# XMUDM/SPEX

Measured on NVIDIA B200. Metric: lightgcn_propagation_gedges_per_s, higher is better.
Workload: dtype f32

## Files before the change

spex_b200/csrc/spmm.cu:

```cuda
#include "common.cuh"
#include <math.h>

namespace spex {

int64_t g_launches = 0;

template <int D>
struct RowShape {
  static_assert(D == 32 || D == 64 || D == 128, "vector path supports D in {32,64,128}");
  static constexpr int LPR = D / 4;
  static constexpr int G = 32 / LPR;
};

template <int D, int U, bool kList, bool kHot = false>
__device__ __forceinline__ float4 warp_row_accumulate(const int32_t* __restrict__ col,
                                                      const float* __restrict__ val,
                                                      const float* __restrict__ X, int64_t start,
                                                      int64_t end, int lane) {
  constexpr int LPR = RowShape<D>::LPR, G = RowShape<D>::G;
  const int grp = lane / LPR, sub = lane % LPR;
  const float* Xs = X + sub * 4;
  float4 acc = f4_zero();
  uint64_t pol_last = 0, pol_first = 0;
  if (kHot) {
// ... 99 lines not shown
      f8 x[U];
      float vv[U];
#pragma unroll
      for (int u = 0; u < U; ++u) {
        const int cc = __shfl_sync(kFull, c, k0 + u, LPR8);
        vv[u] = __shfl_sync(kFull, v, k0 + u, LPR8);
        if (k0 + u < ng) {
          x[u] = gather_row8<D, kHot, kCold>(Xs, cc);
        } else {
          x[u].a = f4_zero();
          x[u].b = f4_zero();
          vv[u] = 0.f;
        }
      }
#pragma unroll
      for (int u = 0; u < U; ++u) f8_fma(acc, vv[u], x[u]);
    }
  }
}

template <int D>
__device__ __forceinline__ void groups_reduce8(f8& acc) {
#pragma unroll
  for (int m = D / 8; m < 32; m <<= 1) {
    f4_add(acc.a, f4_shfl_xor(acc.a, m));
    f4_add(acc.b, f4_shfl_xor(acc.b, m));
  }
}

template <int D, int U, bool kHot>
__device__ __forceinline__ float4 warp_row_accumulate8(const int32_t* __restrict__ col,
                                                       const float* __restrict__ val,
                                                       const float* __restrict__ X, int64_t start,
                                                       int64_t end, int lane) {
  constexpr int LPR8 = D / 8;
  const int grp = lane / LPR8, sub = lane % LPR8;
  const float* Xs = X + sub * 8;
  f8 acc;
  acc.a = f4_zero();
  acc.b = f4_zero();
  int rem = (int)(end - start);
  const int32_t* cp = col + start + lane;
  const float* vp = val + start + lane;
  int c = 0;
  float v = 0.f;
  if (lane < rem) {
    c = ld_stream_s32(cp);
    v = ld_stream_f32(vp);
  }
  while (rem > 0) {
    int cn = 0;
    float vn = 0.f;
    if (lane + 32 < rem) {
      cn = ld_stream_s32(cp + 32);
      vn = ld_stream_f32(vp + 32);
    }
    batch_accumulate8<D, U, kHot>(acc, Xs, c, v, rem, grp);
    c = cn;
    v = vn;
    cp += 32;
    vp += 32;
    rem -= 32;
  }
  groups_reduce8<D>(acc);
  const int src = (lane >> 1) & (LPR8 - 1);
  float4 lo, hi;
  lo.x = __shfl_sync(kFull, acc.a.x, src);
  lo.y = __shfl_sync(kFull, acc.a.y, src);
  lo.z = __shfl_sync(kFull, acc.a.z, src);
  lo.w = __shfl_sync(kFull, acc.a.w, src);
  hi.x = __shfl_sync(kFull, acc.b.x, src);
  hi.y = __shfl_sync(kFull, acc.b.y, src);
  hi.z = __shfl_sync(kFull, acc.b.z, src);
  hi.w = __shfl_sync(kFull, acc.b.w, src);
  return (lane & 1) ? hi : lo;
}

#ifndef SPEX_V8_U
#define SPEX_V8_U 4
#endif
#ifndef SPEX_MASK_U
#define SPEX_MASK_U 2
#endif
#ifndef SPEX_V8_MINB
#define SPEX_V8_MINB 32
#endif
template <int D, bool kHot>
__device__ __forceinline__ float4 warp_row_accumulate8_masked(const int32_t* __restrict__ col,
                                                              const float* __restrict__ val,
                                                              const float* __restrict__ X,
                                                              const uint8_t* __restrict__ nz, int64_t start,
                                                              int64_t end, int lane) {
  constexpr int LPR8 = D / 8;
  constexpr int U = SPEX_MASK_U;
  const int grp = lane / LPR8, sub = lane % LPR8;
  const float* Xs = X + sub * 8;
  f8 acc;
  acc.a = f4_zero();
  acc.b = f4_zero();
  int rem = (int)(end - start);
  const int32_t* cp = col + start + lane;
  const float* vp = val + start + lane;
  constexpr uint32_t kIdMask = kHot ? 0x7fffffffu : 0xffffffffu;
  int c = 0, cn = 0;
  float v = 0.f, vn = 0.f;
  bool on = false;
  if (lane < rem) {
    c = ld_stream_s32(cp);
    v = ld_stream_f32(vp);
  }
  if (lane + 32 < rem) {
    cn = ld_stream_s32(cp + 32);
    vn = ld_stream_f32(vp + 32);
  }
  if (lane < rem) on = nz[(uint32_t)c & kIdMask] != 0;
  while (rem > 0) {
    int c2 = 0;
    float v2 = 0.f;
    if (lane + 64 < rem) {
      c2 = ld_stream_s32(cp + 64);
      v2 = ld_stream_f32(vp + 64);
    }
    bool onn = false;
    if (lane + 32 < rem) onn = nz[(uint32_t)cn & kIdMask] != 0;
    const unsigned act = __ballot_sync(kFull, on);
    unsigned mine = (act >> (grp * LPR8)) & (LPR8 == 32 ? 0xffffffffu : ((1u << LPR8) - 1u));
#pragma unroll 1
    while (__any_sync(kFull, mine != 0)) {
      f8 x[U];
      float vv[U];
#pragma unroll
      for (int u = 0; u < U; ++u) {
        const bool has = mine != 0;
        const int src = grp * LPR8 + (has ? __ffs(mine) - 1 : 0);
        mine &= mine - 1;
        const int cc = __shfl_sync(kFull, c, src);
        vv[u] = __shfl_sync(kFull, v, src);
        if (has) {
          x[u] = gather_row8<D, kHot>(Xs, cc);
        } else {
          x[u].a = f4_zero();
          x[u].b = f4_zero();
          vv[u] = 0.f;
        }
      }
#pragma unroll
      for (int u = 0; u < U; ++u) f8_fma(acc, vv[u], x[u]);
    }
    c = cn;
    v = vn;
    on = onn;
    cn = c2;
    vn = v2;
    cp += 32;
    vp += 32;
    rem -= 32;
  }
#pragma unroll
  for (int m = LPR8; m < 32; m <<= 1) {
    f4_add(acc.a, f4_shfl_xor(acc.a, m));
    f4_add(acc.b, f4_shfl_xor(acc.b, m));
  }
  const int src = (lane >> 1) & (LPR8 - 1);
  float4 lo, hi;
  lo.x = __shfl_sync(kFull, acc.a.x, src);
  lo.y = __shfl_sync(kFull, acc.a.y, src);
  lo.z = __shfl_sync(kFull, acc.a.z, src);
  lo.w = __shfl_sync(kFull, acc.a.w, src);
  hi.x = __shfl_sync(kFull, acc.b.x, src);
  hi.y = __shfl_sync(kFull, acc.b.y, src);
  hi.z = __shfl_sync(kFull, acc.b.z, src);
  hi.w = __shfl_sync(kFull, acc.b.w, src);
  return (lane & 1) ? hi : lo;
}

template <int D, int U, bool kHot, bool kV8, bool kMask = false>
__device__ __forceinline__ float4 row_sum(const int32_t* __restrict__ col, const float* __restrict__ val,
                                          const float* __restrict__ X, int64_t start, int64_t end, int lane,
                                          const uint8_t* __restrict__ nz = nullptr) {
  if (kV8 && kMask) return warp_row_accumulate8_masked<D, kHot>(col, val, X, nz, start, end, lane);
  if (kV8) return warp_row_accumulate8<D, (D >= 64 ? SPEX_V8_U : D / 8), kHot>(col, val, X, start, end, lane);
  return warp_row_accumulate<D, U, false, kHot>(col, val, X, start, end, lane);
}

struct Epilogue {
  float* Y;
  const float* addend;
  float addend_scale;
  float* Z;
  float z_scale;
  float* peer[8];
  int n_peers;
  int64_t peer_row_offset;
  float* mcast;
  const float* pub_src;
  float* pub_mcast;
  float* pub_peer[8];
  int n_pub_peers;
  float* adam_p;
  float* adam_m;
  float* adam_v;
  float adam_b1, adam_b2, adam_eps, adam_step_size, adam_bc2_sqrt;
};

__device__ __forceinline__ void adam_update(float& pp, float gg, float& mm, float& vv, const Epilogue& ep) {
  mm = mm + (gg - mm) * (1.f - ep.adam_b1);
  vv = vv * ep.adam_b2 + (1.f - ep.adam_b2) * gg * gg;
  const float denom = sqrtf(vv) / ep.adam_bc2_sqrt + ep.adam_eps;
  pp = pp - ep.adam_step_size * (mm / denom);
}

template <int D>
__device__ __forceinline__ void row_epilogue(const Epilogue& ep, float4 acc, int64_t row, int lane) {
  constexpr int LPR = RowShape<D>::LPR;
  if (lane < LPR) {
    const int64_t off = row * D + lane * 4;
    if (ep.Y) *reinterpret_cast<float4*>(ep.Y + off) = acc;
    if (ep.mcast) {
      st_multimem_f4(ep.mcast + (row + ep.peer_row_offset) * D + lane * 4, acc);
    } else if (ep.n_peers > 0) {
      const int64_t poff = (row + ep.peer_row_offset) * D + lane * 4;
#pragma unroll
      for (int p = 0; p < 8; ++p)
        if (p < ep.n_peers) *reinterpret_cast<float4*>(ep.peer[p] + poff) = acc;
    }
    float4 z = acc;
    if (ep.Z || ep.adam_p) {
      float4 a = f4_zero();
      if (ep.addend) a = ld_f4(ep.addend + off);
      z.x = (a.x * ep.addend_scale + acc.x) * ep.z_scale;
      z.y = (a.y * ep.addend_scale + acc.y) * ep.z_scale;
      z.z = (a.z * ep.addend_scale + acc.z) * ep.z_scale;
      z.w = (a.w * ep.addend_scale + acc.w) * ep.z_scale;
      if (ep.Z) *reinterpret_cast<float4*>(ep.Z + off) = z;
    }
    float4 pnew = f4_zero();
    if (ep.adam_p) {
      pnew = ld_f4(ep.adam_p + off);
      float4 mm = ld_f4(ep.adam_m + off), vv = ld_f4(ep.adam_v + off);
      adam_update(pnew.x, z.x, mm.x, vv.x, ep);
      adam_update(pnew.y, z.y, mm.y, vv.y, ep);
      adam_update(pnew.z, z.z, mm.z, vv.z, ep);
      adam_update(pnew.w, z.w, mm.w, vv.w, ep);
      *reinterpret_cast<float4*>(ep.adam_p + off) = pnew;
      *reinterpret_cast<float4*>(ep.adam_m + off) = mm;
      *reinterpret_cast<float4*>(ep.adam_v + off) = vv;
    }
    if (ep.pub_src || (ep.adam_p && (ep.pub_mcast || ep.n_pub_peers > 0))) {
      const float4 v = ep.adam_p ? pnew : ld_stream_f4(ep.pub_src + off);
      const int64_t poff = (row + ep.peer_row_offset) * D + lane * 4;
      if (ep.pub_mcast) {
        st_multimem_f4(ep.pub_mcast + poff, v);
      } else {
#pragma unroll
        for (int p = 0; p < 8; ++p)
          if (p < ep.n_pub_peers) *reinterpret_cast<float4*>(ep.pub_peer[p] + poff) = v;
      }
    }
  }
}

#ifndef SPEX_ROWS_PER_CTA
#define SPEX_ROWS_PER_CTA 1
#endif
#ifndef SPEX_U64
#define SPEX_U64 8
#endif
constexpr int kRowsPerCta = SPEX_ROWS_PER_CTA;

template <int D, int U, bool kHot, bool kV8, bool kMask>
__global__ void __launch_bounds__(kRowsPerCta * 32, SPEX_V8_MINB / kRowsPerCta)
spmm_rows_kernel(const int64_t* __restrict__ rowptr, const int32_t* __restrict__ col,
                 const float* __restrict__ val, const float* __restrict__ X, int64_t n_rows,
                 int32_t skip_longer_than, Epilogue ep, const int32_t* __restrict__ row_sel,
                 const uint8_t* __restrict__ nz) {
  const int lane = threadIdx.x & 31;
  int64_t row = (int64_t)blockIdx.x * kRowsPerCta + (threadIdx.x >> 5);
  if (row >= n_rows) return;
  if (row_sel) row = row_sel[row];
  const int64_t start = rowptr[row], end = rowptr[row + 1];
  if (skip_longer_than > 0 && end > start + skip_longer_than) return;
  if (kMask && ep.addend && lane < RowShape<D>::LPR && (lane & 7) == 0)
    asm volatile("prefetch.global.L2 [%0];" ::"l"(ep.addend + row * D + lane * 4));
  const float4 acc = row_sum<D, U, kHot, kV8, kMask>(col, val, X, start, end, lane, nz);
  row_epilogue<D>(ep, acc, row, lane);
}

template <int D, int U, bool kHot, bool kV8, bool kMask>
__global__ void __launch_bounds__(kRowsPerCta * 32, SPEX_V8_MINB / kRowsPerCta)
spmm_seg_list_kernel(const int32_t* __restrict__ col, const float* __restrict__ val,
                     const float* __restrict__ X, const int64_t* __restrict__ seg_start,
                     const int32_t* __restrict__ seg_count, int32_t n_seg, float* __restrict__ partial,
                     const int32_t* __restrict__ seg_sel, const uint8_t* __restrict__ nz) {
  constexpr int LPR = RowShape<D>::LPR;
  const int lane = threadIdx.x & 31;
  int seg = blockIdx.x * kRowsPerCta + (threadIdx.x >> 5);
  if (seg >= n_seg) return;
  if (seg_sel) seg = seg_sel[seg];
  const int64_t start = seg_start[seg];
  const float4 acc = row_sum<D, U, kHot, kV8, kMask>(col, val, X, start, start + seg_count[seg], lane, nz);
  if (lane < LPR) *reinterpret_cast<float4*>(partial + (int64_t)seg * D + lane * 4) = acc;
}

#ifndef SPEX_SEG_HUB_RUN
#define SPEX_SEG_HUB_RUN 8
#endif
#ifndef SPEX_SEG_MID_RUN
#define SPEX_SEG_MID_RUN 2
#endif
constexpr int kHubRun = SPEX_SEG_HUB_RUN, kMidRun = SPEX_SEG_MID_RUN;
static_assert(kHubRun <= 32 && kMidRun <= 32, "a run's segment extents are held one per lane");

template <int D, bool kHot, bool kCold>
__device__ __forceinline__ void seg_run8(const int32_t* __restrict__ col, const float* __restrict__ val,
                                         const float* __restrict__ X, const int64_t* __restrict__ seg_start,
                                         const int32_t* __restrict__ seg_count, int first, int n,
                                         float* __restrict__ partial, int lane) {
  constexpr int LPR8 = D / 8, U = D >= 64 ? SPEX_V8_U : D / 8;
  const int grp = lane / LPR8, sub = lane % LPR8;
  const float* Xs = X + sub * 8;
  int64_t my_start = 0;
  int my_cnt = 0;
  if (lane < n) {
    my_start = seg_start[first + lane];
    my_cnt = seg_count[first + lane];
  }
  int64_t start = __shfl_sync(kFull, my_start, 0);
  int rem = __shfl_sync(kFull, my_cnt, 0);
  int c = 0;
  float v = 0.f;
  if (lane < rem) {
    c = ld_stream_s32(col + start + lane);
    v = ld_stream_f32(val + start + lane);
  }
#pragma unroll 1
  for (int k = 0; k < n; ++k) {
    const int64_t nstart = __shfl_sync(kFull, my_start, (k + 1) & 31);
    const int ncnt = k + 1 < n ? __shfl_sync(kFull, my_cnt, (k + 1) & 31) : 0;
    f8 acc;
    acc.a = f4_zero();
    acc.b = f4_zero();
    int64_t e = start + lane;
#pragma unroll 1
    while (rem > 0) {
      int cn = 0;
      float vn = 0.f;
      if (rem > 32) {
        if (lane + 32 < rem) {
          cn = ld_stream_s32(col + e + 32);
          vn = ld_stream_f32(val + e + 32);
        }
      } else if (lane < ncnt) {
        cn = ld_stream_s32(col + nstart + lane);
        vn = ld_stream_f32(val + nstart + lane);
      }
      batch_accumulate8<D, U, kHot, kCold>(acc, Xs, c, v, rem, grp);
      c = cn;
      v = vn;
      e += 32;
      rem -= 32;
    }
    groups_reduce8<D>(acc);
    if (lane < LPR8) {
      float* p = partial + (int64_t)(first + k) * D + lane * 8;
      st_stream_f4(p, acc.a);
      st_stream_f4(p + 4, acc.b);
    }
    start = nstart;
    rem = ncnt;
  }
}

template <int D, bool kHot>
__global__ void __launch_bounds__(32, SPEX_V8_MINB)
spmm_seg_runs_kernel(const int32_t* __restrict__ col, const float* __restrict__ val, const float* __restrict__ X,
                     const int64_t* __restrict__ seg_start, const int32_t* __restrict__ seg_count, int32_t n_seg,
                     int32_t n_hub_seg, float* __restrict__ partial) {
  const int lane = threadIdx.x;
  const int hub_warps = (n_hub_seg + kHubRun - 1) / kHubRun;
  const int w = blockIdx.x;
  if (w < hub_warps) {
    const int first = w * kHubRun;
    const int n = min(kHubRun, n_hub_seg - first);
    seg_run8<D, kHot, false>(col, val, X, seg_start, seg_count, first, n, partial, lane);
  } else {
    const int first = n_hub_seg + (w - hub_warps) * kMidRun;
    if (first >= n_seg) return;
    const int n = min(kMidRun, n_seg - first);
    seg_run8<D, kHot, kHot>(col, val, X, seg_start, seg_count, first, n, partial, lane);
  }
}

template <int D, int U>
__global__ void __launch_bounds__(kRowsPerCta * 32)
spmm_long_fix_list_kernel(const int32_t* __restrict__ long_rows,
                          const int32_t* __restrict__ long_segptr, const int32_t* __restrict__ row_seg,
                          int32_t n_long, const float* __restrict__ partial, Epilogue ep,
                          const int32_t* __restrict__ slot_sel) {
  const int lane = threadIdx.x & 31;
  int r = blockIdx.x * kRowsPerCta + (threadIdx.x >> 5);
  if (r >= n_long) return;
  if (slot_sel) r = slot_sel[r];
  const float4 acc = warp_row_accumulate<D, U, true>(row_seg, nullptr, partial, long_segptr[r],
                                                     long_segptr[r + 1], lane);
  row_epilogue<D>(ep, acc, (int64_t)long_rows[r], lane);
}

template <int NV>
__global__ void __launch_bounds__(kRowsPerCta * 32)
spmm_rows_generic_kernel(const int64_t* __restrict__ rowptr, const int32_t* __restrict__ col,
                         const float* __restrict__ val, const float* __restrict__ X,
                         int64_t n_rows, int32_t D, Epilogue ep) {
  const int lane = threadIdx.x & 31;
  const int64_t row = (int64_t)blockIdx.x * kRowsPerCta + (threadIdx.x >> 5);
  if (row >= n_rows) return;
  const int64_t start = rowptr[row], end = rowptr[row + 1];
  float4 acc[NV];
#pragma unroll
  for (int v = 0; v < NV; ++v) acc[v] = f4_zero();
  for (int64_t base = start; base < end; base += 32) {
    const int64_t e = base + lane;
    int c = 0;
    float w = 0.f;
    if (e < end) {
      c = ld_stream_s32(col + e);
      w = ld_stream_f32(val + e);
    }
    const int n = (int)((end - base) < 32 ? (end - base) : 32);
    for (int j = 0; j < n; ++j) {
      const int cc = __shfl_sync(kFull, c, j);
      const float ww = __shfl_sync(kFull, w, j);
#pragma unroll
      for (int v = 0; v < NV; ++v) {
        const int d = (lane + 32 * v) * 4;
        if (d < D) f4_fma(acc[v], ww, ld_gather_f4(X + (int64_t)cc * D + d));
      }
    }
  }
#pragma unroll
  for (int v = 0; v < NV; ++v) {
    const int d = (lane + 32 * v) * 4;
    if (d < D) {
      const int64_t off = row * D + d;
      if (ep.Y) *reinterpret_cast<float4*>(ep.Y + off) = acc[v];
      if (ep.mcast) {
        st_multimem_f4(ep.mcast + (row + ep.peer_row_offset) * D + d, acc[v]);
      } else {
        for (int p = 0; p < ep.n_peers; ++p)
          *reinterpret_cast<float4*>(ep.peer[p] + (row + ep.peer_row_offset) * D + d) = acc[v];
      }
      if (ep.Z) {
        float4 a = f4_zero();
        if (ep.addend) a = ld_f4(ep.addend + off);
        float4 z;
        z.x = (a.x * ep.addend_scale + acc[v].x) * ep.z_scale;
        z.y = (a.y * ep.addend_scale + acc[v].y) * ep.z_scale;
        z.z = (a.z * ep.addend_scale + acc[v].z) * ep.z_scale;
        z.w = (a.w * ep.addend_scale + acc[v].w) * ep.z_scale;
        *reinterpret_cast<float4*>(ep.Z + off) = z;
      }
    }
  }
}

static bool g_rows_only = false;

struct RowSubset {
  const int32_t* rows;
  int64_t n_rows;
  const int32_t* long_slots;
  int32_t n_long;
  const int32_t* seg_ids;
  int32_t n_seg;
};

template <int D, int U, bool kHot, bool kV8, bool kMask>
static int launch_vec_h(const int64_t* rowptr, const int32_t* col, const float* val, const float* X,
                        int64_t n_rows, const Epilogue& ep, const spex_long_plan* plan,
                        cudaStream_t st, const RowSubset* sub, const uint8_t* nz) {
  const bool rows_only = g_rows_only;
  const bool has_long = plan && plan->n_long > 0;
  const int64_t n_work = sub ? sub->n_rows : n_rows;
  const int64_t grid = (n_work + kRowsPerCta - 1) / kRowsPerCta;
  if (grid > 0x7fffffffLL) return SPEX_E_TOOBIG;
  if (grid > 0) {
    spmm_rows_kernel<D, U, kHot, kV8, kMask><<<(unsigned)grid, kRowsPerCta * 32, 0, st>>>(
        rowptr, col, val, X, n_work, has_long ? plan->seg_len : 0, ep, sub ? sub->rows : nullptr, nz);
    count_launch();
  }
  if (rows_only) return check_last();
  if (has_long) {
    const int32_t n_seg = sub ? sub->n_seg : plan->n_seg;
    const int32_t n_long = sub ? sub->n_long : plan->n_long;
    const int32_t* seg_sel = sub ? sub->seg_ids : nullptr;
    const int32_t* slot_sel = sub ? sub->long_slots : nullptr;
    if (n_long == 0) return check_last();
    const int gs = (n_seg + kRowsPerCta - 1) / kRowsPerCta;
    const int gf = (n_long + kRowsPerCta - 1) / kRowsPerCta;
    if (kV8 && !kMask && !sub && plan->n_hub_seg > 0) {
      const int n_mid = n_seg - plan->n_hub_seg;
      const int gr = (plan->n_hub_seg + kHubRun - 1) / kHubRun + (n_mid + kMidRun - 1) / kMidRun;
      spmm_seg_runs_kernel<D, kHot><<<gr, 32, 0, st>>>(col, val, X, plan->seg_start, plan->seg_count, n_seg,
                                                       plan->n_hub_seg, plan->partial);
    } else {
      spmm_seg_list_kernel<D, U, kHot, kV8, kMask><<<gs, kRowsPerCta * 32, 0, st>>>(
          col, val, X, plan->seg_start, plan->seg_count, n_seg, plan->partial, seg_sel, nz);
    }
    spmm_long_fix_list_kernel<D, U><<<gf, kRowsPerCta * 32, 0, st>>>(
        plan->long_rows, plan->long_segptr, plan->row_seg, n_long, plan->partial, ep, slot_sel);
    count_launch(2);
  }
  return check_last();
}

template <int D, int U>
static int launch_vec(const int64_t* rowptr, const int32_t* col, const float* val, const float* X,
                      int64_t n_rows, const Epilogue& ep, const spex_long_plan* plan,
                      cudaStream_t st, const RowSubset* sub, const uint8_t* nz) {
  const bool v8 = (reinterpret_cast<uintptr_t>(X) & 31u) == 0;
  const bool hot = plan && (plan->flags & SPEX_PLAN_COL_HOTBIT);
  if (nz && v8) {
    if (hot) return launch_vec_h<D, U, true, true, true>(rowptr, col, val, X, n_rows, ep, plan, st, sub, nz);
    return launch_vec_h<D, U, false, true, true>(rowptr, col, val, X, n_rows, ep, plan, st, sub, nz);
  }
  if (hot) {
    if (v8) return launch_vec_h<D, U, true, true, false>(rowptr, col, val, X, n_rows, ep, plan, st, sub, nullptr);
    return launch_vec_h<D, U, true, false, false>(rowptr, col, val, X, n_rows, ep, plan, st, sub, nullptr);
  }
  if (v8) return launch_vec_h<D, U, false, true, false>(rowptr, col, val, X, n_rows, ep, plan, st, sub, nullptr);
  return launch_vec_h<D, U, false, false, false>(rowptr, col, val, X, n_rows, ep, plan, st, sub, nullptr);
}

int spmm_launch(const int64_t* rowptr, const int32_t* col, const float* val, const float* X,
                int64_t n_rows, int32_t D, const Epilogue& ep, const spex_long_plan* plan,
                cudaStream_t st, const RowSubset* sub = nullptr, const uint8_t* nz = nullptr) {
  SPEX_RETURN_IF(!rowptr || !X || n_rows < 0, SPEX_E_BADARG);
  SPEX_RETURN_IF(n_rows > 0 && (!col || !val), SPEX_E_BADARG);
  SPEX_RETURN_IF(D <= 0 || (D & 3) || D > 512, SPEX_E_BADDIM);
  SPEX_RETURN_IF(!aligned16(X) || !aligned16(ep.Y) || !aligned16(ep.Z) || !aligned16(ep.addend),
                 SPEX_E_ALIGN);
  SPEX_RETURN_IF(plan && (plan->flags & ~SPEX_PLAN_COL_HOTBIT), SPEX_E_BADARG);
  if (plan && plan->n_long > 0) {
    SPEX_RETURN_IF(plan->seg_len < 32 || !plan->long_rows || !plan->long_segptr ||
                       !plan->partial || plan->n_seg < plan->n_long,
                   SPEX_E_BADARG);
    SPEX_RETURN_IF(!plan->seg_start || !plan->seg_count || !plan->row_seg, SPEX_E_BADARG);
    SPEX_RETURN_IF(plan->n_hub_seg < 0 || plan->n_hub_seg > plan->n_seg, SPEX_E_BADARG);
    SPEX_RETURN_IF(!aligned16(plan->partial), SPEX_E_ALIGN);
  }
  if (n_rows == 0) return 0;
  switch (D) {
    case 32: return launch_vec<32, 4>(rowptr, col, val, X, n_rows, ep, plan, st, sub, nz);
    case 64: return launch_vec<64, SPEX_U64>(rowptr, col, val, X, n_rows, ep, plan, st, sub, nz);
    case 128: return launch_vec<128, 8>(rowptr, col, val, X, n_rows, ep, plan, st, sub, nz);
    default: break;
  }
  SPEX_RETURN_IF(sub != nullptr, SPEX_E_BADDIM);
  SPEX_RETURN_IF(plan && (plan->flags & SPEX_PLAN_COL_HOTBIT), SPEX_E_BADDIM);
  SPEX_RETURN_IF(ep.pub_src != nullptr || ep.adam_p != nullptr, SPEX_E_BADDIM);
  const int64_t grid = (n_rows + kRowsPerCta - 1) / kRowsPerCta;
  if (grid > 0x7fffffffLL) return SPEX_E_TOOBIG;
  const int nv = (D + 127) / 128;
  switch (nv) {
    case 1: spmm_rows_generic_kernel<1><<<(unsigned)grid, kRowsPerCta * 32, 0, st>>>(rowptr, col, val, X, n_rows, D, ep); break;
    case 2: spmm_rows_generic_kernel<2><<<(unsigned)grid, kRowsPerCta * 32, 0, st>>>(rowptr, col, val, X, n_rows, D, ep); break;
    case 3: spmm_rows_generic_kernel<3><<<(unsigned)grid, kRowsPerCta * 32, 0, st>>>(rowptr, col, val, X, n_rows, D, ep); break;
    default: spmm_rows_generic_kernel<4><<<(unsigned)grid, kRowsPerCta * 32, 0, st>>>(rowptr, col, val, X, n_rows, D, ep); break;
  }
  count_launch();
  return check_last();
}

__global__ void copy_f4_kernel(const float4* __restrict__ src, float4* __restrict__ dst, int64_t n4) {
  int64_t i = (int64_t)blockIdx.x * blockDim.x + threadIdx.x;
  const int64_t stride = (int64_t)gridDim.x * blockDim.x;
  for (; i < n4; i += stride) dst[i] = src[i];
}

struct PeerTables {
  float* peer[8];
  int n_peers;
};
__global__ void __launch_bounds__(256)
push_rows_kernel(const float4* __restrict__ src, int64_t n4, int64_t dst_off4, PeerTables pt) {
  int64_t i = (int64_t)blockIdx.x * blockDim.x + threadIdx.x;
  const int64_t stride = (int64_t)gridDim.x * blockDim.x;
  const int rot = blockIdx.x % pt.n_peers;
  for (; i < n4; i += stride) {
    const float4 v = ld_stream_f4(reinterpret_cast<const float*>(src + i));
#pragma unroll
    for (int p = 0; p < 8; ++p) {
      if (p < pt.n_peers) {
        int q = p + rot;
        if (q >= pt.n_peers) q -= pt.n_peers;
        reinterpret_cast<float4*>(pt.peer[q])[dst_off4 + i] = v;
      }
    }
  }
}

__global__ void __launch_bounds__(256)
mcast_rows_kernel(const float4* __restrict__ src, int64_t n4, float* __restrict__ mcast_dst) {
  int64_t i = (int64_t)blockIdx.x * blockDim.x + threadIdx.x;
  const int64_t stride = (int64_t)gridDim.x * blockDim.x;
  for (; i < n4; i += stride)
    st_multimem_f4(mcast_dst + 4 * i, ld_stream_f4(reinterpret_cast<const float*>(src + i)));
}

__global__ void gather_scale_kernel(const float* __restrict__ src, const int64_t* __restrict__ idx,
                                    const float* __restrict__ scale, float divisor,
                                    float* __restrict__ out, int64_t n) {
  int64_t i = (int64_t)blockIdx.x * blockDim.x + threadIdx.x;
  const int64_t stride = (int64_t)gridDim.x * blockDim.x;
  for (; i < n; i += stride) {
    float v = idx ? src[idx[i]] : src[i];
    if (scale) v *= scale[i];
    if (divisor != 1.f) v = v / divisor;
    out[i] = v;
  }
}

__device__ __forceinline__ uint32_t edge_draw(uint64_t seed, uint32_t r, uint32_t c) {
  return (uint32_t)(splitmix64(seed ^ (((uint64_t)r << 32) | c)) >> 40);
}

constexpr int kDropChunk = 1024;
constexpr int kDropUnroll = 4;

template <bool kT, bool kTpos>
__global__ void __launch_bounds__(256)
edge_dropout_kernel(const int64_t* __restrict__ rowptr, const int32_t* __restrict__ col,
                    const float* __restrict__ val, const int64_t* __restrict__ tpos, int64_t n_rows,
                    int64_t row_offset, uint64_t seed, float keep_prob, float* __restrict__ val_out,
                    float* __restrict__ valT_out) {
  uint32_t k_min = 0, k_hi = 1u << 24;
  while (k_min < k_hi) {
    const uint32_t mid = (k_min + k_hi) >> 1;
    if (__float2int_rz(__fadd_rn(__uint2float_rn(mid) * 0x1p-24f, keep_prob)) != 0) k_hi = mid; else k_min = mid + 1;
  }
  const bool divide = keep_prob != 1.f;
  const int lane = threadIdx.x & (kWarp - 1);
  const int64_t warps = (int64_t)gridDim.x * (blockDim.x / kWarp);
  const int64_t e_end = __ldg(rowptr + n_rows);
  for (int64_t c0 = __ldg(rowptr) + ((int64_t)blockIdx.x * (blockDim.x / kWarp) + threadIdx.x / kWarp) * kDropChunk;
       c0 < e_end; c0 += warps * kDropChunk) {
    int64_t lo = 0, hi = n_rows;
    while (hi - lo > 1) {
      const int64_t mid = (lo + hi) >> 1;
      if (__ldg(rowptr + mid) <= c0) lo = mid; else hi = mid;
    }
    int64_t row = lo;
    int32_t row_end = (int32_t)(__ldg(rowptr + row + 1) - c0);
    const int n = (int)min((int64_t)kDropChunk, e_end - c0);
    const int32_t* cc = col + c0;
    const float* vc = val + c0;
    float* oc = val_out + c0;
    float* ot = kT ? valT_out + c0 : nullptr;
    for (int i0 = lane; i0 < n; i0 += kDropUnroll * kWarp) {
      uint32_t cv[kDropUnroll];
      float v[kDropUnroll], vt[kDropUnroll];
#pragma unroll
      for (int k = 0; k < kDropUnroll; ++k) {
        const int i = i0 + k * kWarp;
        if (i < n) {
          cv[k] = (uint32_t)ld_stream_s32(cc + i) & 0x7fffffffu;
          v[k] = ld_stream_f32(vc + i);
          if (kT && kTpos) vt[k] = __ldg(val + __ldcs(tpos + c0 + i));
        }
      }
#pragma unroll
      for (int k = 0; k < kDropUnroll; ++k) {
        const int i = i0 + k * kWarp;
        if (i >= n) break;
        while (row_end <= i) row_end = (int32_t)(__ldg(rowptr + (++row) + 1) - c0);
        const uint32_t r = (uint32_t)(row + row_offset);
        const float q = divide ? v[k] / keep_prob : v[k];
        __stcs(oc + i, edge_draw(seed, r, cv[k]) >= k_min ? q : v[k] * 0.f);
        if (kT) {
          const float w = kTpos ? vt[k] : v[k];
          const float qt = !kTpos ? q : divide ? w / keep_prob : w;
          __stcs(ot + i, edge_draw(seed, cv[k], r) >= k_min ? qt : w * 0.f);
        }
      }
    }
  }
}

// ... 319 lines not shown
```

spex_b200/ops.py:

```python
from __future__ import annotations

import ctypes as C
from typing import Optional

import numpy as np
import torch

from . import _capi
from ._capi import LongPlan, call, ptr, stream_ptr
from .graph import CSRGraph, DEFAULT_SEG_LEN


class _Workspaces:

    def __init__(self):
        self.enabled = False
        self.buf = {}
        self.dirty = {}

    def get(self, name, shape, device, zero=False):
        key = (name, tuple(shape), str(device))
        t = self.buf.get(key) if self.enabled else None
        if t is None:
            t = (torch.zeros if zero else torch.empty)(*shape, dtype=torch.float32, device=device)
            if self.enabled:
                self.buf[key] = t
                self.dirty[key] = []
        elif zero:
            D = shape[-1]
            for rows in self.dirty[key]:
                call("spex_clear_rows_f32", ptr(t), ptr(rows), rows.numel(), D, stream_ptr())
            self.dirty[key] = []
        return t, key

    def mark(self, key, *row_lists):
        if self.enabled and key in self.dirty:
            self.dirty[key].extend(r for r in row_lists if r is not None and r.numel())

    def clear(self):
        self.buf.clear()
        self.dirty.clear()


workspaces = _Workspaces()


def enable_persistent_workspaces(on: bool = True):
    workspaces.enabled = bool(on)
    if not on:
        workspaces.clear()


def _scatter_workspace(total, device):
    nbytes = int(call("spex_scatter_workspace_bytes", int(total)))
    if nbytes == 0:
        return None, 0
    key = ("scatter_ws", str(device))
    t = workspaces.buf.get(key) if workspaces.enabled else None
    if t is None or t.numel() < nbytes:
        t = torch.empty(nbytes, dtype=torch.uint8, device=device)
        if workspaces.enabled:
            workspaces.buf[key] = t
    return t, nbytes


def _need_cuda(*tensors):
    for t in tensors:
        if t is not None and not t.is_cuda:
            raise RuntimeError(
                "spex_b200 runs on sm_100a only: got a CPU tensor (there is no CPU fallback path)"
            )


def _f32c(t: torch.Tensor) -> torch.Tensor:
    if t.dtype != torch.float32:
        raise TypeError(f"expected float32, got {t.dtype}")
    return t if t.is_contiguous() else t.contiguous()


def _i64c(t: torch.Tensor, device) -> torch.Tensor:
    if not torch.is_tensor(t):
        t = torch.as_tensor(np.asarray(t))
    t = t.to(device=device, dtype=torch.int64, non_blocking=True)
    return t if t.is_contiguous() else t.contiguous()


class DeviceGraph:

    interleave_split = 0

    def __init__(self, rowptr, col, val, n_cols: int, tpos=None, seg_len: int = DEFAULT_SEG_LEN,
                 row_offset: int = 0, symmetric: bool = True, D_hint: int = 64, col_hot: bool = False,
                 values_symmetric: bool = False):
        _need_cuda(rowptr, col, val)
        assert rowptr.dtype == torch.int64 and col.dtype == torch.int32 and val.dtype == torch.float32
        self.rowptr, self.col, self.val = rowptr, col, val
        self.n_rows = rowptr.numel() - 1
        self.n_cols = int(n_cols)
        self.nnz = col.numel()
        self.tpos = tpos
        self.row_offset = int(row_offset)
        self.symmetric = symmetric
        self.values_symmetric = values_symmetric
        self.device = val.device
        self.seg_len = int(seg_len)
        self._plan_struct = None
        self._plan_D = 0
        self._plan_tensors = None
        self.col_hot = False
        if col_hot:
            self.col_hot = True
        self._build_plan(D_hint)

    @classmethod
    def from_host(cls, g: CSRGraph, device, seg_len: int = DEFAULT_SEG_LEN, D_hint: int = 64):
        dev = torch.device(device)
        rowptr = torch.from_numpy(np.ascontiguousarray(g.rowptr)).to(dev)
        col = torch.from_numpy(np.ascontiguousarray(g.col)).to(dev)
        val = torch.from_numpy(np.ascontiguousarray(g.val)).to(dev)
        tpos = None if g.tpos is None else torch.from_numpy(np.ascontiguousarray(g.tpos)).to(dev)
        return cls(rowptr, col, val, g.n_cols, tpos, seg_len, g.row_offset, D_hint=D_hint)

    @classmethod
    def from_sparse_coo(cls, A: torch.Tensor, device, seg_len: int = DEFAULT_SEG_LEN):
        A = A.coalesce()
        idx = A.indices()
        n_rows, n_cols = A.shape
        dev = torch.device(device)
        rows = idx[0].to(dev)
        counts = torch.bincount(rows, minlength=n_rows)
        rowptr = torch.zeros(n_rows + 1, dtype=torch.int64, device=dev)
        torch.cumsum(counts, 0, out=rowptr[1:])
        col = idx[1].to(dev).to(torch.int32)
        val = A.values().to(dev).to(torch.float32)
        return cls(rowptr, col, val, n_cols, None, seg_len)

    L2_WINDOW_BYTES = 16 << 20
    MIN_CB_COLS = 1024
    HUB_EDGES_PER_BLOCK = 16

    def _build_plan(self, D: int):
        self.__dict__.update(self.long_row_plan(self.rowptr, self.col, self.n_cols, self.seg_len, D))
        self._plan_D = 0

    @classmethod
    def long_row_plan(cls, rowptr: torch.Tensor, col: torch.Tensor, n_cols: int, seg_len: int, D: int) -> dict:
        if seg_len < 32:
            raise ValueError("seg_len must be >= 32")
        dev = rowptr.device
        nnz = col.numel()
        deg = rowptr[1:] - rowptr[:-1]
        long_rows = torch.nonzero(deg > seg_len).flatten()
        n_long = int(long_rows.numel())
        ldeg = deg[long_rows]
        is_hub = torch.zeros_like(ldeg, dtype=torch.bool)
        parts_start, parts_cnt, parts_row = [], [], []
        n_hub_cells = 0
        if n_cols * D * 4 > 4 * cls.L2_WINDOW_BYTES:
            import os as _os
            win = int(_os.environ.get("SPEX_L2_WINDOW_MB", 0)) << 20 or cls.L2_WINDOW_BYTES
            epb = int(_os.environ.get("SPEX_HUB_EPB", 0)) or cls.HUB_EDGES_PER_BLOCK
            cb_cols = max(win // (D * 4), cls.MIN_CB_COLS)
            n_cb = (n_cols + cb_cols - 1) // cb_cols
            is_hub = ldeg >= epb * n_cb
            hub_slots = torch.nonzero(is_hub).flatten()
            if hub_slots.numel():
                hrows = long_rows[hub_slots]
                nh = hrows.numel()
                lo = rowptr[hrows].unsqueeze(1).expand(nh, n_cb + 1).clone()
                hi = rowptr[hrows + 1].unsqueeze(1).expand(nh, n_cb + 1).clone()
                target = (torch.arange(n_cb + 1, device=dev, dtype=torch.int64) * cb_cols).unsqueeze(0)
                steps = int(ldeg.max().item()).bit_length() + 1
                last = nnz - 1
                for _ in range(steps):
                    mid = (lo + hi) >> 1
                    go = ((col[mid.clamp(max=last)] & 0x7FFFFFFF).to(torch.int64) < target) & (lo < hi)
                    lo = torch.where(go, mid + 1, lo)
                    hi = torch.where(go, hi, mid)
                pos = lo
                del lo, hi, mid, go
                cs = pos[:, :-1].t().reshape(-1)
                cc = (pos[:, 1:] - pos[:, :-1]).t().reshape(-1)
                cr = hub_slots.repeat(n_cb)
                keep = cc > 0
                parts_start.append(cs[keep]); parts_cnt.append(cc[keep]); parts_row.append(cr[keep])
                n_hub_cells = int(parts_cnt[0].numel())
        mid_slots = torch.nonzero(~is_hub).flatten()
        mrows = long_rows[mid_slots]
        parts_start.append(rowptr[mrows]); parts_cnt.append(deg[mrows]); parts_row.append(mid_slots)
        cell_start = torch.cat(parts_start)
        cell_cnt = torch.cat(parts_cnt)
        cell_row = torch.cat(parts_row)
        pieces = (cell_cnt + seg_len - 1) // seg_len
        seg_cell = torch.repeat_interleave(torch.arange(cell_cnt.numel(), device=dev), pieces)
        first = torch.cumsum(pieces, 0) - pieces
        piece_idx = torch.arange(seg_cell.numel(), device=dev) - first[seg_cell]
        seg_start = cell_start[seg_cell] + piece_idx * seg_len
        seg_end = torch.minimum(seg_start + seg_len, (cell_start + cell_cnt)[seg_cell])
        seg_row = cell_row[seg_cell]
        n_seg = int(seg_start.numel())
        if n_seg >= 2 ** 31:
            raise ValueError("too many long-row segments")
        order = torch.sort(seg_row * (nnz + 1) + seg_start, stable=True).indices
        counts = torch.bincount(seg_row, minlength=n_long)
        segptr = torch.zeros(n_long + 1, dtype=torch.int64, device=dev)
        torch.cumsum(counts, 0, out=segptr[1:])
        return {"n_long": n_long, "n_seg": n_seg, "n_hub": int(is_hub.sum()),
                "n_hub_seg": int(pieces[:n_hub_cells].sum()),
                "long_rows": long_rows.to(torch.int32), "long_segptr": segptr.to(torch.int32),
                "seg_start": seg_start.contiguous(), "seg_count": (seg_end - seg_start).to(torch.int32).contiguous(),
                "row_seg": order.to(torch.int32).contiguous()}

    HOT_L2_BYTES = 48 << 20

    def mark_hot_columns(self, D: int, col_degree: Optional[torch.Tensor] = None,
                         budget_bytes: Optional[int] = None) -> int:
        if self.col_hot:
            return -1
        import os as _os
        budget = budget_bytes if budget_bytes is not None else (
            int(_os.environ.get("SPEX_HOT_L2_MB", 0)) << 20 or self.HOT_L2_BYTES)
        n_hot = min(budget // (D * 4), self.n_cols)
        if self.n_cols * D * 4 <= 2 * budget or n_hot <= 0 or D not in (32, 64, 128):
            return 0
        if col_degree is None:
            if self.n_rows != self.n_cols:
                raise ValueError("column degrees are needed for a non-square graph")
            col_degree = self.rowptr[1:] - self.rowptr[:-1]
        thr = torch.topk(col_degree, n_hot).values[-1]
        hot = col_degree >= torch.clamp(thr, min=2)
        if int(hot.sum()) > 2 * n_hot:
            return 0
        chunk = 1 << 28
        int_min = -(2 ** 31)
        for s0 in range(0, self.nnz, chunk):
            c = self.col[s0: s0 + chunk]
            c.bitwise_or_(hot[c.long()].to(torch.int32) * int_min)
        self.col_hot = True
        self._plan_D = 0
        return int(hot.sum())

    def clean_col(self) -> torch.Tensor:
        return (self.col & 0x7FFFFFFF) if self.col_hot else self.col

    def plan(self, D: int):
        if self.n_long == 0 and not self.col_hot:
            return None
        if self._plan_D != D:
            flags = 1 if self.col_hot else 0
            if self.n_long == 0:
                st = LongPlan(self.seg_len, 0, 0, flags)
                self._plan_tensors = None
            else:
                partial = torch.empty(self.n_seg * D, dtype=torch.float32, device=self.device)
                st = LongPlan(self.seg_len, self.n_long, self.n_seg, flags, self.long_rows.data_ptr(),
                              self.long_segptr.data_ptr(), partial.data_ptr(), self.seg_start.data_ptr(),
                              self.seg_count.data_ptr(), self.row_seg.data_ptr(), self.n_hub_seg)
                self._plan_tensors = partial
            self._plan_struct = st
            self._plan_D = D
        return C.byref(self._plan_struct)

    def _edge_positions(self, rows: torch.Tensor):
        a = self.rowptr[rows]
        cnt = self.rowptr[rows + 1] - a
        total = int(cnt.sum().item())
        first = torch.cumsum(cnt, 0) - cnt
        pos = torch.repeat_interleave(a - first, cnt, output_size=total) + torch.arange(total, device=self.device)
        return pos, total

    def degree_sum(self, rows: torch.Tensor) -> int:
        return int((self.rowptr[rows + 1] - self.rowptr[rows]).sum().item())

    def neighbors(self, rows: torch.Tensor) -> torch.Tensor:
        pos, total = self._edge_positions(rows)
        if total == 0:
            return torch.empty(0, dtype=torch.int64, device=self.device)
        c = self.col[pos]
        if self.col_hot:
            c = c & 0x7FFFFFFF
        return torch.unique(c.to(torch.int64))

    def row_subset(self, rows: torch.Tensor):
        rows = rows.to(torch.int64)
        r32 = rows.to(torch.int32).contiguous()
        if self.n_long == 0:
            return r32, None, None
        deg = self.rowptr[rows + 1] - self.rowptr[rows]
        lr = rows[deg > self.seg_len]
        if lr.numel() == 0:
            return r32, None, None
        slots = torch.searchsorted(self.long_rows.to(torch.int64), lr)
        segptr = self.long_segptr.to(torch.int64)
        a = segptr[slots]
        cnt = segptr[slots + 1] - a
        total = int(cnt.sum().item())
        first = torch.cumsum(cnt, 0) - cnt
        pos = torch.repeat_interleave(a - first, cnt, output_size=total) + torch.arange(total, device=self.device)
        seg_ids = self.row_seg[pos]
        return r32, slots.to(torch.int32).contiguous(), seg_ids.to(torch.int32).contiguous()

    def with_values(self, val: torch.Tensor, symmetric: bool) -> "DeviceGraph":
        g = object.__new__(DeviceGraph)
        g.__dict__.update(self.__dict__)
        g.val = val
        g.symmetric = symmetric
        return g

    def transposed_values(self, val: torch.Tensor) -> torch.Tensor:
        if self.tpos is None:
            raise RuntimeError("graph has no transpose map (tpos)")
        out = torch.empty_like(val)
        call("spex_gather_f32", ptr(val), ptr(self.tpos), None, 1.0, ptr(out), self.nnz, stream_ptr())
        return out

    def dropout_values(self, keep_mask: torch.Tensor, keep_prob: float) -> torch.Tensor:
        scale = keep_mask.to(self.device, torch.float32).contiguous()
        out = torch.empty_like(self.val)
        call("spex_gather_f32", ptr(self.val), None, ptr(scale), float(keep_prob), ptr(out), self.nnz,
             stream_ptr())
        return out

    def device_dropout_values(self, seed: int, keep_prob: float):
        if self.tpos is None and not self.values_symmetric:
            raise RuntimeError("edge dropout needs the transpose map of the adjacency or bit-symmetric values; "
                               "build the graph through spex_b200.dataloader (getCSR) or synthetic.build_norm_adj_device")
        val = torch.empty_like(self.val)
        valT = torch.empty_like(self.val)
        call("spex_edge_dropout_f32", ptr(self.rowptr), ptr(self.col), ptr(self.val), ptr(self.tpos), self.n_rows,
             self.row_offset, int(seed), float(keep_prob), ptr(val), ptr(valT), stream_ptr())
        return val, valT

    def to_sparse_coo(self) -> torch.Tensor:
        deg = self.rowptr[1:] - self.rowptr[:-1]
        rows = torch.repeat_interleave(torch.arange(self.n_rows, device=self.device), deg)
        idx = torch.stack([rows + self.row_offset, self.clean_col().to(torch.int64)])
        return torch.sparse_coo_tensor(idx, self.val, (self.n_rows, self.n_cols), is_coalesced=True)


def spmm(g: DeviceGraph, X: torch.Tensor, Y: Optional[torch.Tensor] = None,
         addend: Optional[torch.Tensor] = None, addend_scale: float = 1.0,
         Z: Optional[torch.Tensor] = None, z_scale: float = 1.0, val: Optional[torch.Tensor] = None):
    _need_cuda(X)
    X = _f32c(X)
    D = X.shape[1]
    if X.shape[0] != g.n_cols:
        raise ValueError(f"X has {X.shape[0]} rows, graph has {g.n_cols} columns")
    if Y is None and Z is None:
        Y = torch.empty(g.n_rows, D, dtype=torch.float32, device=X.device)
    v = g.val if val is None else val
    call("spex_spmm_csr_f32", ptr(g.rowptr), ptr(g.col), ptr(v), ptr(X), g.n_rows, D, ptr(Y),
         ptr(addend), float(addend_scale), ptr(Z), float(z_scale), g.plan(D), stream_ptr())
    return Y if Y is not None else Z


def nonzero_mask(n: int, rows: torch.Tensor) -> torch.Tensor:
    m = torch.zeros(n, dtype=torch.uint8, device=rows.device)
    m[rows] = 1
    return m


def spmm_rows(g: DeviceGraph, X: torch.Tensor, subset, Y: Optional[torch.Tensor] = None,
              addend: Optional[torch.Tensor] = None, addend_scale: float = 1.0,
              Z: Optional[torch.Tensor] = None, z_scale: float = 1.0, val: Optional[torch.Tensor] = None,
              x_nonzero: Optional[torch.Tensor] = None):
    _need_cuda(X)
    X = _f32c(X)
    D = X.shape[1]
    if X.shape[0] != g.n_cols:
        raise ValueError(f"X has {X.shape[0]} rows, graph has {g.n_cols} columns")
    if Y is None and Z is None:
        raise ValueError("spmm_rows writes into caller-provided Y and/or Z")
    rows, slots, segs = subset if subset is not None else (None, None, None)
    v = g.val if val is None else val
    if x_nonzero is not None and (x_nonzero.dtype != torch.uint8 or x_nonzero.numel() != g.n_cols):
        raise ValueError("x_nonzero must be uint8 [n_cols]")
    call("spex_spmm_csr_rows_f32", ptr(g.rowptr), ptr(g.col), ptr(v), ptr(X), g.n_rows, D, ptr(rows),
         -1 if rows is None else rows.numel(), ptr(slots), 0 if slots is None else slots.numel(), ptr(segs),
         0 if segs is None else segs.numel(), ptr(x_nonzero), ptr(Y), ptr(addend), float(addend_scale), ptr(Z),
         float(z_scale), g.plan(D), stream_ptr())


SPARSE_INPUT_MAX_EDGE_FRAC = 0.3
SUBSET_MAX_EDGE_FRAC = 0.5
EXPAND_MAX_EDGE_FRAC = 0.02


def receptive_rows(graph: DeviceGraph, S: torch.Tensor, K: int):
    R = [None] * (K + 1)
    if K < 1 or graph.degree_sum(S) > SUBSET_MAX_EDGE_FRAC * graph.nnz:
        return R
    R[K] = S
    for k in range(K - 1, 0, -1):
        if graph.degree_sum(R[k + 1]) > EXPAND_MAX_EDGE_FRAC * graph.nnz:
            break
        cand = torch.unique(torch.cat([S, graph.neighbors(R[k + 1])]))
        if graph.degree_sum(cand) > SUBSET_MAX_EDGE_FRAC * graph.nnz:
            break
        R[k] = cand
    return R


class _PropagateMeanRows(torch.autograd.Function):

    @staticmethod
    def forward(ctx, table, graph: DeviceGraph, K: int, val, valT, S):
        _need_cuda(table)
        E0 = _f32c(table)
        N, D = E0.shape
        R = receptive_rows(graph, S, K)
        subs = [None if r is None else graph.row_subset(r) for r in R]
        out = torch.empty_like(E0) if not workspaces.enabled else workspaces.get("prop_out", E0.shape, E0.device)[0]
        tmp = [workspaces.get("prop_tmp0", E0.shape, E0.device)[0] if K >= 2 else None,
               workspaces.get("prop_tmp1", E0.shape, E0.device)[0] if K >= 3 else None]
        v = graph.val if val is None else val
        inv = 1.0 / float(K + 1)
        X = E0
        for k in range(1, K + 1):
            last = k == K
            Y = None if last else tmp[(k - 1) & 1]
            kw = dict(Y=Y, addend=E0 if k == 1 else out, addend_scale=1.0, Z=out, z_scale=inv if last else 1.0, val=v)
            if subs[k] is None:
                spmm(graph, X, **kw)
            else:
                spmm_rows(graph, X, subs[k], **kw)
            X = Y
        ctx.graph, ctx.K, ctx.valT, ctx.subs, ctx.R = graph, K, (v if valT is None else valT), subs, R
        return out

    @staticmethod
    def backward(ctx, g):
        graph, K, subs, R = ctx.graph, ctx.K, ctx.subs, ctx.R
        g = _f32c(g)
        N, D = g.shape
        dE0 = torch.empty_like(g) if not workspaces.enabled else workspaces.get("prop_dE0", g.shape, g.device)[0]
        tmp = [workspaces.get("prop_tmp0", g.shape, g.device)[0] if K >= 2 else None,
               workspaces.get("prop_tmp1", g.shape, g.device)[0] if K >= 3 else None]
        inv = 1.0 / float(K + 1)
        X = g
        x_rows = R[K]
        for j in range(1, K + 1):
            last = j == K
            sub = subs[K - j] if j < K else None
            kw = dict(addend=g, addend_scale=1.0, z_scale=inv if last else 1.0, val=ctx.valT)
            mask = None
            if x_rows is not None and graph.degree_sum(x_rows) <= SPARSE_INPUT_MAX_EDGE_FRAC * graph.nnz:
                mask = nonzero_mask(N, x_rows)
            if sub is None:
                Z = dE0 if last else tmp[(j - 1) & 1]
                if mask is None:
                    spmm(graph, X, Z=Z, **kw)
                else:
                    spmm_rows(graph, X, None, Z=Z, x_nonzero=mask, **kw)
                x_rows = None
            else:
                Z, zkey = workspaces.get(f"prop_bwd_rows{j}", g.shape, g.device, zero=True)
                spmm_rows(graph, X, sub, Z=Z, x_nonzero=mask, **kw)
                workspaces.mark(zkey, R[K - j])
                x_rows = R[K - j]
            X = Z
        return dE0, None, None, None, None, None


class _PropagateMean(torch.autograd.Function):

    @staticmethod
    def forward(ctx, table, graph: DeviceGraph, K: int, val, valT):
        _need_cuda(table)
        E0 = _f32c(table)
        N, D = E0.shape
        out = torch.empty_like(E0) if not workspaces.enabled else workspaces.get("prop_out", E0.shape, E0.device)[0]
        tmp0 = workspaces.get("prop_tmp0", E0.shape, E0.device)[0] if K >= 2 else None
        tmp1 = workspaces.get("prop_tmp1", E0.shape, E0.device)[0] if K >= 3 else None
        v = graph.val if val is None else val
        call("spex_propagate_mean_f32", ptr(graph.rowptr), ptr(graph.col), ptr(v), ptr(E0), N, D, K,
             ptr(out), ptr(tmp0), ptr(tmp1), graph.plan(D), stream_ptr())
        ctx.graph, ctx.K, ctx.valT = graph, K, (v if valT is None else valT)
        return out

    @staticmethod
    def backward(ctx, g):
        graph, K = ctx.graph, ctx.K
        g = _f32c(g)
        N, D = g.shape
        dE0 = torch.empty_like(g) if not workspaces.enabled else workspaces.get("prop_dE0", g.shape, g.device)[0]
        tmp0 = workspaces.get("prop_tmp0", g.shape, g.device)[0] if K >= 2 else None
        tmp1 = workspaces.get("prop_tmp1", g.shape, g.device)[0] if K >= 3 else None
        call("spex_propagate_mean_bwd_f32", ptr(graph.rowptr), ptr(graph.col), ptr(ctx.valT), ptr(g),
# ... 367 lines not shown
```

Baseline: 41.43.

## Add packed small-cell hub path and refine hub classification by column-block span

Adds a hub_cells8 device path for warps whose hub cells all have tiny edge counts. Several cells are packed across lane groups, partial sums are parked in shared memory and reduced per cell, so lanes are not left idle on small cells. The host planner now marks a row as a hub based on the number of column blocks it actually spans rather than the total block count. Within each column block, hub cells are sorted by descending count so small cells cluster into the same warps. This adds shared-memory traffic, extra shuffles and branchy control flow, and the edits to row classification change how work is split between the hub and mid paths.

```diff
diff --git a/spex_b200/csrc/spmm.cu b/spex_b200/csrc/spmm.cu
--- a/spex_b200/csrc/spmm.cu
+++ b/spex_b200/csrc/spmm.cu
@@ -425,6 +425,13 @@
   if (lane < LPR) *reinterpret_cast<float4*>(partial + (int64_t)seg * D + lane * 4) = acc;
 }
 
+#ifndef SPEX_HUB_SMALL
+#define SPEX_HUB_SMALL 8
+#endif
+#ifndef SPEX_HUB_U
+#define SPEX_HUB_U 2
+#endif
+constexpr int kHubSmall = SPEX_HUB_SMALL;
 #ifndef SPEX_SEG_HUB_RUN
 #define SPEX_SEG_HUB_RUN 8
 #endif
@@ -494,18 +501,134 @@
   }
 }
 
+__device__ __forceinline__ void f8_add(f8& a, const f8& b) {
+  f4_add(a.a, b.a);
+  f4_add(a.b, b.b);
+}
+
+template <int D, bool kHot>
+__device__ __forceinline__ void hub_cells8(const int32_t* __restrict__ col, const float* __restrict__ val,
+                                           const float* __restrict__ X, const int64_t* __restrict__ seg_start,
+                                           const int32_t* __restrict__ seg_count, int first, int n,
+                                           float* __restrict__ partial, int lane, f8 (*park)[32]) {
+  constexpr int LPR8 = D / 8, G = 32 / LPR8, U = D >= 64 ? SPEX_V8_U : D / 8, UG = SPEX_HUB_U;
+  const int grp = lane / LPR8, sub = lane % LPR8;
+  const float* Xs = X + sub * 8;
+  int64_t my_start = 0;
+  int my_cnt = 0;
+  if (lane < n) {
+    my_start = seg_start[first + lane];
+    my_cnt = seg_count[first + lane];
+  }
+  int k = grp, off = 0;
+  int64_t start = __shfl_sync(kFull, my_start, k);
+  int cnt = __shfl_sync(kFull, my_cnt, k);
+  if (k >= n) cnt = 0;
+  int c = 0;
+  float v = 0.f;
+  if (sub < cnt) {
+    c = ld_stream_s32(col + start + sub);
+    v = ld_stream_f32(val + start + sub);
+  }
+  f8 acc;
+  acc.a = f4_zero();
+  acc.b = f4_zero();
+#pragma unroll 1
+  while (__any_sync(kFull, cnt > 0)) {
+    const int r = (off & 31) / LPR8;
+    const bool r_done = off + 32 >= cnt;
+    const int r_last = min(G - 1, (cnt - 1) / LPR8);
+    const bool cell_done = r_done && r >= r_last;
+    const int nk = cell_done ? k + G : k;
+    const int noff = !r_done ? off + 32 : cell_done ? 0 : LPR8 * (r + 1);
+    const int64_t s_next = __shfl_sync(kFull, my_start, nk & 31);
+    const int c_next = __shfl_sync(kFull, my_cnt, nk & 31);
+    const int64_t nstart = cell_done ? s_next : start;
+    const int ncnt = cell_done ? (nk < n ? c_next : 0) : cnt;
+    int cn = 0;
+    float vn = 0.f;
+    if (sub < ncnt - noff) {
+      cn = ld_stream_s32(col + nstart + noff + sub);
+      vn = ld_stream_f32(val + nstart + noff + sub);
+    }
+    const int ng = cnt - off;
+#pragma unroll
+    for (int k0 = 0; k0 < LPR8; k0 += UG) {
+      if (!__any_sync(kFull, k0 < ng)) break;
+      f8 x[UG];
+      float vv[UG];
+#pragma unroll
+      for (int u = 0; u < UG; ++u) {
+        const int cc = __shfl_sync(kFull, c, k0 + u, LPR8);
+        vv[u] = __shfl_sync(kFull, v, k0 + u, LPR8);
+        if (k0 + u < ng) x[u] = gather_row8<D, kHot, false>(Xs, cc);
+      }
+#pragma unroll
+      for (int u = 0; u < UG; ++u)
+        if (k0 + u < ng) f8_fma(acc, vv[u], x[u]);
+    }
+    if (r_done && cnt > 0) {
+      const int rem_l = cnt - ((cnt - 1) & ~31);
+      const int nmax = min(rem_l, LPR8);
+      if (rem_l < 32 && rem_l - LPR8 * r < (nmax + U - 1) / U * U) {
+        f8 z;
+        z.a = f4_zero();
+        z.b = f4_zero();
+        f8_add(acc, z);
+      }
+      park[r][lane] = acc;
+      acc.a = f4_zero();
+      acc.b = f4_zero();
+      if (cell_done) {
+        f8 a[G];
+#pragma unroll
+        for (int q = 0; q < G; ++q) {
+          if (q <= r_last) {
+            a[q] = park[q][lane];
+          } else {
+            a[q].a = f4_zero();
+            a[q].b = f4_zero();
+          }
+        }
+#pragma unroll
+        for (int m = 1; m < G; m <<= 1)
+#pragma unroll
+          for (int q = 0; q < G; q += 2 * m) f8_add(a[q], a[q + m]);
+        float* p = partial + (int64_t)(first + k) * D + sub * 8;
+        st_stream_f4(p, a[0].a);
+        st_stream_f4(p + 4, a[0].b);
+      }
+    }
+    k = nk;
+    off = noff;
+    start = nstart;
+    cnt = ncnt;
+    c = cn;
+    v = vn;
+  }
+}
+
 template <int D, bool kHot>
 __global__ void __launch_bounds__(32, SPEX_V8_MINB)
 spmm_seg_runs_kernel(const int32_t* __restrict__ col, const float* __restrict__ val, const float* __restrict__ X,
                      const int64_t* __restrict__ seg_start, const int32_t* __restrict__ seg_count, int32_t n_seg,
                      int32_t n_hub_seg, float* __restrict__ partial) {
+  __shared__ f8 park[D >= 64 ? 32 / (D / 8) : 1][32];
   const int lane = threadIdx.x;
   const int hub_warps = (n_hub_seg + kHubRun - 1) / kHubRun;
   const int w = blockIdx.x;
   if (w < hub_warps) {
     const int first = w * kHubRun;
     const int n = min(kHubRun, n_hub_seg - first);
-    seg_run8<D, kHot, false>(col, val, X, seg_start, seg_count, first, n, partial, lane);
+    bool small = false;
+    if constexpr (D >= 64) {
+      const int cnt = lane < n ? seg_count[first + lane] : 0;
+      small = __reduce_max_sync(kFull, (unsigned)cnt) <= kHubSmall;
+    }
+    if (small)
+      hub_cells8<D, kHot>(col, val, X, seg_start, seg_count, first, n, partial, lane, park);
+    else
+      seg_run8<D, kHot, false>(col, val, X, seg_start, seg_count, first, n, partial, lane);
   } else {
     const int first = n_hub_seg + (w - hub_warps) * kMidRun;
     if (first >= n_seg) return;
diff --git a/spex_b200/ops.py b/spex_b200/ops.py
--- a/spex_b200/ops.py
+++ b/spex_b200/ops.py
@@ -162,7 +162,9 @@
             epb = int(_os.environ.get("SPEX_HUB_EPB", 0)) or cls.HUB_EDGES_PER_BLOCK
             cb_cols = max(win // (D * 4), cls.MIN_CB_COLS)
             n_cb = (n_cols + cb_cols - 1) // cb_cols
-            is_hub = ldeg >= epb * n_cb
+            first_cb = (col[rowptr[long_rows]] & 0x7FFFFFFF).to(torch.int64) // cb_cols
+            last_cb = (col[rowptr[long_rows + 1] - 1] & 0x7FFFFFFF).to(torch.int64) // cb_cols
+            is_hub = ldeg >= epb * (last_cb - first_cb + 1)
             hub_slots = torch.nonzero(is_hub).flatten()
             if hub_slots.numel():
                 hrows = long_rows[hub_slots]
@@ -183,7 +185,10 @@
                 cc = (pos[:, 1:] - pos[:, :-1]).t().reshape(-1)
                 cr = hub_slots.repeat(n_cb)
                 keep = cc > 0
-                parts_start.append(cs[keep]); parts_cnt.append(cc[keep]); parts_row.append(cr[keep])
+                cs, cc, cr = cs[keep], cc[keep], cr[keep]
+                blk = torch.nonzero(keep).flatten() // nh
+                order = torch.sort(blk * (nnz + 1) + (nnz - cc), stable=True).indices
+                parts_start.append(cs[order]); parts_cnt.append(cc[order]); parts_row.append(cr[order])
                 n_hub_cells = int(parts_cnt[0].numel())
         mid_slots = torch.nonzero(~is_hub).flatten()
         mrows = long_rows[mid_slots]
```

Result: no change. 41.64, median of 6 (+0.5%).
